# second-state/qwen3_asr_rs

Hardware: NVIDIA H100
Metric: real-time factor (audio-sec/wall-sec) Qwen3-ASR-0.6B 30s clips (higher is better)
Workload: dtype f32 (bf16 weights, fp32-exact activations)

## Files before the change

### qwen3_asr_rs_b200/csrc/attention_f32.cu

```cuda
#include "internal.h"

namespace asrb {

namespace af32 {

static constexpr int QT = 32, KT = 64, THREADS = 128, PS = KT + 4;

template <int HD, bool OFF>
__global__ void __launch_bounds__(THREADS, 2) attn_f32_kernel(AttnParams p) {
    constexpr int NG = HD / 64;
    extern __shared__ __align__(16) float sm[];
    float* Qt = sm;
    float* Kt = Qt + HD * QT;
    float* Vs = Kt + HD * KT;
    float* Ps = Vs + KT * HD;
    const int seg = blockIdx.z, h = blockIdx.y;
    const int q0 = p.seg_q0[seg], len = p.seg_len[seg];
    const int pos0 = OFF ? p.seg_pos0[seg] : 0;
    const int nqt = (len + QT - 1) / QT;
    const int gkv = h / p.group;
    const int tid = threadIdx.x, tx = tid & 15, ty = tid >> 4;
    const float* kbase; const float* vbase;
    if (p.keys_in_rows) {
        kbase = p.k + (size_t)q0 * p.ldk + (size_t)gkv * p.head_stride;
        vbase = p.v + (size_t)q0 * p.ldk + (size_t)gkv * p.head_stride;
    } else {
        kbase = p.k + (size_t)seg * p.seg_stride + (size_t)gkv * p.head_stride;
        vbase = p.v + (size_t)seg * p.seg_stride + (size_t)gkv * p.head_stride;
    }
    const int npass = p.causal ? 2 : 1;
    for (int pass = 0; pass < npass; ++pass) {
// ... 139 lines not shown
    }
}

template <int HD> static size_t smem_bytes() { return (size_t)(HD * QT + HD * KT + KT * HD + QT * PS) * sizeof(float); }

}

bool launch_attention_f32(const AttnParams& p, int hd, cudaStream_t st) {
    using namespace af32;
    if (p.nseg <= 0 || p.max_len <= 0) return true;
    if ((p.ldq % 4) || (p.ldk % 4) || (p.head_stride % 4) || (p.seg_stride % 4)) return false;
    const int nqt_max = (p.max_len + QT - 1) / QT;
    dim3 grid(p.causal ? (nqt_max + 1) / 2 : nqt_max, p.nheads, p.nseg);
    auto run = [&](auto kern, size_t smem) {
        ASRB_CUDA_CHECK(cudaFuncSetAttribute(kern, cudaFuncAttributeMaxDynamicSharedMemorySize, (int)smem));
        kern<<<grid, THREADS, smem, st>>>(p);
    };
    const bool off = p.seg_pos0 != nullptr;
    if (off && !p.causal) return false;
    if (hd == 64) run(off ? attn_f32_kernel<64, true> : attn_f32_kernel<64, false>, smem_bytes<64>());
    else if (hd == 128) run(off ? attn_f32_kernel<128, true> : attn_f32_kernel<128, false>, smem_bytes<128>());
    else return false;
    ASRB_CUDA_CHECK(cudaGetLastError());
    return true;
}

}
```

### qwen3_asr_rs_b200/csrc/common.cuh

```cuda
#pragma once
#include <cuda_runtime.h>
#include <cuda_bf16.h>
#include <stdint.h>
#include <stdexcept>
#include <string>

namespace asrb {

struct Error : public std::runtime_error {
    int code;
    Error(int c, const std::string& m) : std::runtime_error(m), code(c) {}
};

#define ASRB_CUDA_CHECK(expr)                                                              \
    do {                                                                                   \
        cudaError_t _e = (expr);                                                           \
        if (_e != cudaSuccess)                                                             \
            throw ::asrb::Error(2, std::string(#expr) + " failed: " + cudaGetErrorString(_e) + \
                                       " (" __FILE__ ":" + std::to_string(__LINE__) + ")"); \
    } while (0)

#define ASRB_REQUIRE(cond, code, msg)                                          \
    do {                                                                       \
        if (!(cond)) throw ::asrb::Error((code), std::string(msg));            \
// ... 50 lines not shown
    if (lane == 0) scratch[w] = v;
    __syncthreads();
    float r = (lane < nw) ? scratch[lane] : 0.f;
    r = warp_sum(r);
    return r;
}
__device__ __forceinline__ float block_max(float v, float* scratch) {
    int lane = threadIdx.x & 31, w = threadIdx.x >> 5, nw = (blockDim.x + 31) >> 5;
    v = warp_max(v);
    __syncthreads();
    if (lane == 0) scratch[w] = v;
    __syncthreads();
    float r = (lane < nw) ? scratch[lane] : -INFINITY;
    r = warp_max(r);
    return r;
}

__device__ __forceinline__ float lse_rescale(float s, float m, float M) { return m == M ? s : s * expf(m - M); }
__device__ __forceinline__ void lse_fold(float v, int row, float& best_v, int& best_i, float& best_s) {
    if (v > best_v) { best_s = lse_rescale(best_s, best_v, v) + 1.f; best_v = v; best_i = row; }
    else best_s += expf(v - best_v);
}
__device__ __forceinline__ float lse_merge(float m, float s, float om, float os) {
    const float M = fmaxf(m, om);
    return lse_rescale(s, m, M) + lse_rescale(os, om, M);
}

constexpr int TK_MAX = 8;
struct TopK { float v[TK_MAX]; int i[TK_MAX]; };
__device__ __forceinline__ bool tk_before(float a, int ai, float b, int bi) { return a > b || (a == b && ai < bi); }
// ... 146 lines not shown
```

### qwen3_asr_rs_b200/csrc/elementwise.cu

```cuda
#include "internal.h"

namespace asrb {

__global__ void conv1_gelu_kernel(const float* __restrict__ mel, const int* __restrict__ chunk_clip,
                                  const int* __restrict__ chunk_f0, const int64_t* __restrict__ foff,
                                  const int64_t* __restrict__ frames, int n_mels, int W, int OH, int OW,
                                  const float* __restrict__ w, const float* __restrict__ bias, int dsh,
                                  int cpad, bf16* __restrict__ out, size_t plane_stride) {
    extern __shared__ float rows[];
    const int chunk = blockIdx.y, oh = blockIdx.x;
    const int clip = chunk_clip[chunk], f0 = chunk_f0[chunk];
    const int F = (int)frames[clip];
    const float* mp = mel + (size_t)n_mels * foff[clip];
    for (int idx = threadIdx.x; idx < 3 * (W + 2); idx += blockDim.x) {
        int kh = idx / (W + 2), wi = idx - kh * (W + 2);
        int h = 2 * oh + kh - 1, wcol = wi - 1;
        float v = 0.f;
        if (h >= 0 && h < n_mels && wcol >= 0 && wcol < W && f0 + wcol < F) v = mp[(size_t)h * F + f0 + wcol];
        rows[idx] = v;
    }
    __syncthreads();
    const int c = threadIdx.x;
    if (c >= dsh) return;
    float wk[9];
// ... 20 lines not shown
    int W = d.conv_w[0], OH = d.conv_h[1], OW = d.conv_w[1];
    dim3 grid(OH, n_chunks);
    int threads = ((d.c.downsample_hidden_size + 31) / 32) * 32;
    size_t smem = 3 * (W + 2) * sizeof(float);
    conv1_gelu_kernel<<<grid, threads, smem, st>>>(mel, d_chunk_clip, d_chunk_f0, d_foff, d_frames,
                                                   d.c.num_mel_bins, W, OH, OW, m.conv1_w, m.conv1_b,
                                                   d.c.downsample_hidden_size, d.cpad, out_s3, plane_stride);
    ASRB_CUDA_CHECK(cudaGetLastError());
}

__global__ void layernorm_s3_kernel(const float* __restrict__ x, const float* __restrict__ w,
                                    const float* __restrict__ b, int dim, float eps, bf16* __restrict__ out,
                                    size_t plane_stride) {
    __shared__ float red[32];
    const size_t row = blockIdx.x;
    const float* xr = x + row * dim;
    float s = 0.f;
    for (int i = threadIdx.x; i < dim; i += blockDim.x) s += xr[i];
    const float mean = block_sum(s, red) / dim;
    float v = 0.f;
    for (int i = threadIdx.x; i < dim; i += blockDim.x) { float dlt = xr[i] - mean; v = fmaf(dlt, dlt, v); }
    const float var = block_sum(v, red) / dim;
    const float rstd = 1.0f / sqrtf(var + eps);
    for (int i = threadIdx.x; i < dim; i += blockDim.x)
        store_split3(out, plane_stride, row * dim + i, (xr[i] - mean) * rstd * w[i] + b[i]);
}
__global__ void rmsnorm_s3_kernel(const float* __restrict__ x, const float* __restrict__ w, int dim, float eps,
                                  bf16* __restrict__ out, size_t plane_stride) {
    __shared__ float red[32];
    const size_t row = blockIdx.x;
    const float* xr = x + row * dim;
    float s = 0.f;
    for (int i = threadIdx.x; i < dim; i += blockDim.x) s = fmaf(xr[i], xr[i], s);
    const float var = block_sum(s, red) / dim;
    const float r = 1.0f / sqrtf(var + eps);
    for (int i = threadIdx.x; i < dim; i += blockDim.x)
        store_split3(out, plane_stride, row * dim + i, (xr[i] * r) * w[i]);
}
void launch_layernorm_s3(const float* x, const float* w, const float* b, int rows, int dim, float eps,
                         bf16* out_s3, size_t plane_stride, cudaStream_t st) {
    if (rows <= 0) return;
    layernorm_s3_kernel<<<rows, 128, 0, st>>>(x, w, b, dim, eps, out_s3, plane_stride);
    ASRB_CUDA_CHECK(cudaGetLastError());
}
void launch_rmsnorm_s3(const float* x, const float* w, int rows, int dim, float eps, bf16* out_s3,
                       size_t plane_stride, cudaStream_t st) {
    if (rows <= 0) return;
    rmsnorm_s3_kernel<<<rows, 128, 0, st>>>(x, w, dim, eps, out_s3, plane_stride);
    ASRB_CUDA_CHECK(cudaGetLastError());
}

__global__ void embed_inject_kernel(const bf16* __restrict__ embed, int hidden, const int* __restrict__ ids,
                                    const int* __restrict__ audio_row, const float* __restrict__ audio,
                                    float* __restrict__ out) {
    const size_t row = blockIdx.x;
    const int ar = audio_row[row];
    float* o = out + row * hidden;
    if (ar >= 0) {
        const float* a = audio + (size_t)ar * hidden;
        for (int i = threadIdx.x; i < hidden; i += blockDim.x) o[i] = a[i];
    } else {
        const bf16* e = embed + (size_t)ids[row] * hidden;
        for (int i = threadIdx.x; i < hidden; i += blockDim.x) o[i] = __bfloat162float(e[i]);
    }
}
void launch_embed_inject(const bf16* embed, int hidden, const int* d_ids, const int* d_audio_row,
                         const float* audio, int rows, float* out, cudaStream_t st) {
    if (rows <= 0) return;
    embed_inject_kernel<<<rows, 256, 0, st>>>(embed, hidden, d_ids, d_audio_row, audio, out);
    ASRB_CUDA_CHECK(cudaGetLastError());
}

template <bool FAN>
__global__ void qk_norm_rope_kernel(const float* __restrict__ qkv, const int* __restrict__ row_seq,
                                    const int* __restrict__ row_pos, const float* __restrict__ qnorm,
                                    const float* __restrict__ knorm, float eps,
                                    const float* __restrict__ rope_cos, const float* __restrict__ rope_sin,
                                    int nq, int nkv, int hd, float* __restrict__ q_out,
                                    float* __restrict__ kcache, float* __restrict__ vcache,
                                    size_t cache_seq_stride, int max_ctx, FanOut fan) {
    extern __shared__ float sh[];
    float* ys = sh;
    float* red = sh + hd;
    const size_t row = blockIdx.x;
    const int head = blockIdx.y, d = threadIdx.x;
    const int qkv_dim = (nq + 2 * nkv) * hd;
    const float x = qkv[row * qkv_dim + (size_t)head * hd + d];
    const int seq = row_seq[row], pos = row_pos[row];
    const int nfan = FAN && pos < fan.P[seq] ? fan.n[seq] : 0;
    const int* fslots = FAN ? fan.slots + fan.off[seq] : nullptr;
    if (head >= nq + nkv) {
        const size_t o = ((size_t)(head - nq - nkv) * max_ctx + pos) * hd + d;
        vcache[seq * cache_seq_stride + o] = x;
        for (int j = 0; j < nfan; ++j) vcache[(size_t)fslots[j] * cache_seq_stride + o] = x;
        return;
    }
    const float* nw = head < nq ? qnorm : knorm;
    const float var = block_sum(x * x, red) / hd;
    const float y = (x * (1.0f / sqrtf(var + eps))) * nw[d];
    ys[d] = y;
    __syncthreads();
// ... 3 lines not shown
    const float o = y * c + rot * s;
    if (head < nq) q_out[row * ((size_t)nq * hd) + (size_t)head * hd + d] = o;
    else {
        const size_t ko = ((size_t)(head - nq) * max_ctx + pos) * hd + d;
        kcache[seq * cache_seq_stride + ko] = o;
        for (int j = 0; j < nfan; ++j) kcache[(size_t)fslots[j] * cache_seq_stride + ko] = o;
    }
}
void launch_qk_norm_rope(const float* qkv, int rows, const int* d_row_seq, const int* d_row_pos,
                         const float* qnorm, const float* knorm, float eps, const float* rope_cos,
                         const float* rope_sin, int nq, int nkv, int hd, float* q_out, float* kcache,
                         float* vcache, size_t cache_seq_stride, int max_ctx, cudaStream_t st, const FanOut* fan) {
    if (rows <= 0) return;
    dim3 grid(rows, nq + 2 * nkv);
    const size_t smem = (hd + 32) * sizeof(float);
    if (fan) qk_norm_rope_kernel<true><<<grid, hd, smem, st>>>(qkv, d_row_seq, d_row_pos, qnorm, knorm, eps, rope_cos, rope_sin,
                                                               nq, nkv, hd, q_out, kcache, vcache, cache_seq_stride, max_ctx, *fan);
    else qk_norm_rope_kernel<false><<<grid, hd, smem, st>>>(qkv, d_row_seq, d_row_pos, qnorm, knorm, eps, rope_cos, rope_sin,
                                                            nq, nkv, hd, q_out, kcache, vcache, cache_seq_stride, max_ctx, FanOut{});
    ASRB_CUDA_CHECK(cudaGetLastError());
}

}
```

### qwen3_asr_rs_b200/csrc/gemm_simt.cu

```cuda
#include "internal.h"
#include "epilogue.cuh"

namespace asrb {

static constexpr int BM = 64, BN = 64, BK = 16, CHUNK_K = 256;

__global__ void __launch_bounds__(256) gemm_simt_kernel(GemmA A, const bf16* __restrict__ W, int N, GemmEpi E) {
    __shared__ float As[BK][BM + 4];
    __shared__ float Ws[BK][BN + 4];
    const int m0 = blockIdx.y * BM, n0 = blockIdx.x * BN;
    const int tid = threadIdx.x;
    const int tx = tid & 15, ty = tid >> 4;
    float acc[4][4], sum[4][4];
#pragma unroll
    for (int i = 0; i < 4; ++i)
#pragma unroll
        for (int j = 0; j < 4; ++j) acc[i][j] = sum[i][j] = 0.f;
    for (int k0 = 0; k0 < A.K; k0 += BK) {
#pragma unroll
        for (int i = 0; i < 4; ++i) {
            int idx = tid + i * 256;
            int r = idx >> 4, kk = idx & 15;
            int m = m0 + r, k = k0 + kk;
            As[kk][r] = (m < A.M && k < A.K) ? load_a(A, m, k) : 0.f;
// ... 30 lines not shown
            int n = n0 + tx * 4 + j;
            if (n >= N) continue;
            epi_store2(E, N, m, n, sum[i][j], sum[i][j + 1], n + 1 < N);
        }
    }
}

void launch_gemm_simt(const GemmA& A, const bf16* W, int N, const GemmEpi& E, cudaStream_t st) {
    dim3 grid((N + BN - 1) / BN, (A.M + BM - 1) / BM);
    if (A.M <= 0 || N <= 0) return;
    gemm_simt_kernel<<<grid, 256, 0, st>>>(A, W, N, E);
    ASRB_CUDA_CHECK(cudaGetLastError());
}

std::atomic<int64_t> g_gemm_simt_fallbacks{0}, g_gemm_tc_launches{0};

void launch_gemm(const GemmA& A, const bf16* W, int N, const GemmEpi& E, int impl, cudaStream_t st) {
    if (impl == GEMM_TC) {
        if (launch_gemm_tc(A, W, N, E, st)) { g_gemm_tc_launches += 1; return; }
        g_gemm_simt_fallbacks += 1;
    }
    launch_gemm_simt(A, W, N, E, st);
}

}
```

### qwen3_asr_rs_b200/csrc/gemm_tc.cu

```cuda
#include <cuda.h>
#include <algorithm>
#include <cstring>
#include <map>
#include <tuple>
#include "internal.h"
#include "epilogue.cuh"
#include "wgmma.cuh"

namespace asrb {
namespace tc {

static constexpr int BM = 128, BN = 128, BK = 64, STAGES = 3;
static constexpr int TILE_A_BYTES = BM * BK * 2;
static constexpr int TILE_B_BYTES = BN * BK * 2;
static constexpr int STAGE_BYTES = 3 * TILE_A_BYTES + TILE_B_BYTES;
static constexpr int NTHREADS = 384;
static constexpr int CONS_WARPS = 8;
static constexpr int SLAB_LD = 40;
static constexpr int CH = 4;

struct ConvGeom { int OH, OW, box_h, tiles_per_chunk, kblk_per_tap, a_box_bytes; };

template <int A_MODE, int EPI_MODE>
__global__ void __launch_bounds__(NTHREADS, 1)
// ... 2 lines not shown
    extern __shared__ __align__(1024) uint8_t smem_raw[];
    uint8_t* smem = reinterpret_cast<uint8_t*>((reinterpret_cast<uintptr_t>(smem_raw) + 1023) & ~(uintptr_t)1023);
    uint64_t* full = reinterpret_cast<uint64_t*>(smem + STAGES * STAGE_BYTES);
    uint64_t* empty = full + STAGES;
    float* epi_slab = reinterpret_cast<float*>(smem + STAGES * STAGE_BYTES + 256);
    const int warp = threadIdx.x >> 5, lane = threadIdx.x & 31;
    const int num_kb = K / BK / splits;
    const int n_items = tiles_m * tiles_n * splits;

    if (threadIdx.x == 0) {
        for (int i = 0; i < STAGES; ++i) { mbar_init(&full[i], 1); mbar_init(&empty[i], CONS_WARPS); }
        asm volatile("fence.mbarrier_init.release.cluster;" ::: "memory");
        asm volatile("prefetch.tensormap [%0];" ::"l"(&mapA) : "memory");
        asm volatile("prefetch.tensormap [%0];" ::"l"(&mapB) : "memory");
    }
    __syncthreads();

    auto item_coords = [&](int item, int& n0, int& m0, int& chunk, int& oh0, int& z) {
        const int nt = item % tiles_n; int rest = item / tiles_n;
        const int mt = rest % tiles_m; z = rest / tiles_m;
        n0 = nt * BN; m0 = mt * BM; chunk = 0; oh0 = 0;
        if (A_MODE == 1) { chunk = mt / cg.tiles_per_chunk; oh0 = (mt % cg.tiles_per_chunk) * cg.box_h; }
    };

    if (warp == 0 && lane == 0) {
        const uint32_t a_bytes = (A_MODE == 0) ? (uint32_t)TILE_A_BYTES : (uint32_t)cg.a_box_bytes;
        const uint32_t stage_tx = (uint32_t)nplanes * a_bytes + (uint32_t)TILE_B_BYTES;
        uint32_t kg = 0;
        for (int item = blockIdx.x; item < n_items; item += gridDim.x) {
            int n0, m0, chunk, oh0, z;
// ... 51 lines not shown
                    }
                    mr[i] = (m >= 0 && ncol) ? m : -1;
                    if (mr[i] >= 0) in[i] = epi_fetch4<EPI_MODE>(E, N, (int)mr[i], n);
                }
#pragma unroll
                for (int i = 0; i < 4; ++i)
                    if (mr[i] >= 0) epi_store4<EPI_MODE>(E, N, (int)mr[i], n, v[i], bias4, in[i]);
                __syncwarp();
            }
        }
    }
}

template <int MODE>
__global__ void __launch_bounds__(256) splitk_reduce_kernel(const float* __restrict__ ws, int S, int M, int N, GemmEpi E) {
    const int n8 = N / 8;
    const int idx = blockIdx.x * blockDim.x + threadIdx.x;
    if (idx >= M * n8) return;
    const int m = idx / n8, n = (idx - m * n8) * 8;
    float v[8];
#pragma unroll
    for (int i = 0; i < 8; ++i) v[i] = 0.f;
    for (int sp = 0; sp < S; ++sp) {
        const float* src = ws + ((size_t)sp * M + m) * N + n;
        const float4 a = *reinterpret_cast<const float4*>(src), b = *reinterpret_cast<const float4*>(src + 4);
        v[0] += a.x; v[1] += a.y; v[2] += a.z; v[3] += a.w; v[4] += b.x; v[5] += b.y; v[6] += b.z; v[7] += b.w;
    }
    epi_store8<MODE>(E, N, m, n, v);
}

typedef CUresult (*EncodeTiledFn)(CUtensorMap*, CUtensorMapDataType, cuuint32_t, void*, const cuuint64_t*, const cuuint64_t*,
                                  const cuuint32_t*, const cuuint32_t*, CUtensorMapInterleave, CUtensorMapSwizzle,
                                  CUtensorMapL2promotion, CUtensorMapFloatOOBfill);
static EncodeTiledFn get_encode() {
    static EncodeTiledFn fn = nullptr;
    if (!fn) {
        void* p = nullptr;
        cudaDriverEntryPointQueryResult qr;
        ASRB_CUDA_CHECK(cudaGetDriverEntryPoint("cuTensorMapEncodeTiled", &p, cudaEnableDefault, &qr));
        ASRB_REQUIRE(p != nullptr && qr == cudaDriverEntryPointSuccess, ASRB_ERR_CUDA, "cuTensorMapEncodeTiled unavailable");
        fn = (EncodeTiledFn)p;
    }
    return fn;
// ... 91 lines not shown
    cuuint64_t bs[1] = {(cuuint64_t)A.K * 2};
    cuuint32_t bb[2] = {(cuuint32_t)BK, (cuuint32_t)BN};
    const CUtensorMap mapB = cached_map(W, 2, bd, bs, bb);
    ConvGeom cg{};
    const size_t smem = smem_bytes();
    const int tiles_m = pl.tiles_m, tiles_n = pl.tiles_n;
    if (A.mode == A_PLAIN) {
        cuuint64_t ad[3] = {(cuuint64_t)A.K, (cuuint64_t)A.M, (cuuint64_t)3};
        cuuint64_t as[2] = {(cuuint64_t)A.lda * 2, (cuuint64_t)A.plane_stride * 2};
        cuuint32_t ab[3] = {(cuuint32_t)BK, (cuuint32_t)BM, 1};
        const CUtensorMap mapA = cached_map(A.a, 3, ad, as, ab);
        if (pl.splits > 1) {
            GemmEpi P;
            P.out_f32 = E.splitk_ws; P.ldo = N;
            ASRB_CUDA_CHECK(cudaFuncSetAttribute(gemm_tc_kernel<0, EPI_PLAIN>, cudaFuncAttributeMaxDynamicSharedMemorySize, (int)smem));
            gemm_tc_kernel<0, EPI_PLAIN><<<pl.grid, NTHREADS, smem, st>>>(mapA, mapB, A.M, N, A.K, A.nplanes, tiles_m, tiles_n, pl.splits, cg, P);
            const int work = A.M * (N / 8);
            if (E.mode == EPI_PLAIN) splitk_reduce_kernel<EPI_PLAIN><<<(work + 255) / 256, 256, 0, st>>>(E.splitk_ws, pl.splits, A.M, N, E);
            else splitk_reduce_kernel<EPI_CONVOUT><<<(work + 255) / 256, 256, 0, st>>>(E.splitk_ws, pl.splits, A.M, N, E);
            ASRB_CUDA_CHECK(cudaGetLastError());
            if (E.extra_launches) *E.extra_launches += 1;
            return true;
        }
#define ASRB_TC_LAUNCH(AM, EM)                                                                                         \
    {                                                                                                                  \
        ASRB_CUDA_CHECK(cudaFuncSetAttribute(gemm_tc_kernel<AM, EM>, cudaFuncAttributeMaxDynamicSharedMemorySize, (int)smem)); \
        gemm_tc_kernel<AM, EM><<<pl.grid, NTHREADS, smem, st>>>(mapA, mapB, A.M, N, A.K, A.nplanes, tiles_m, tiles_n, 1, cg, E); \
    }
        if (E.mode == EPI_PLAIN) ASRB_TC_LAUNCH(0, EPI_PLAIN)
        else if (E.mode == EPI_SWIGLU) ASRB_TC_LAUNCH(0, EPI_SWIGLU)
        else ASRB_TC_LAUNCH(0, EPI_CONVOUT)
    } else {
        const int chunks = A.M / (A.OH * A.OW);
        cg.OH = A.OH; cg.OW = A.OW; cg.box_h = pl.box_h;
        cg.tiles_per_chunk = (A.OH + cg.box_h - 1) / cg.box_h; cg.kblk_per_tap = A.cpad / BK;
        cg.a_box_bytes = A.OW * cg.box_h * BK * 2;
        cuuint64_t ad[5] = {(cuuint64_t)A.cpad, (cuuint64_t)A.Wh, (cuuint64_t)A.Hh, (cuuint64_t)chunks * 4, 3};
        cuuint64_t as[4] = {(cuuint64_t)A.cpad * 2, (cuuint64_t)A.Wh * A.cpad * 2, (cuuint64_t)A.Hh * A.Wh * A.cpad * 2,
                            (cuuint64_t)A.plane_stride * 2};
        cuuint32_t ab[5] = {(cuuint32_t)BK, (cuuint32_t)A.OW, (cuuint32_t)cg.box_h, 1, 1};
        const CUtensorMap mapA = cached_map(A.a, 5, ad, as, ab);
        if (E.mode == EPI_CONV_PARITY) ASRB_TC_LAUNCH(1, EPI_CONV_PARITY)
        else ASRB_TC_LAUNCH(1, EPI_CONV_FEAT)
#undef ASRB_TC_LAUNCH
    }
    ASRB_CUDA_CHECK(cudaGetLastError());
    return true;
}

}
```

### qwen3_asr_rs_b200/csrc/internal.h

```cpp
#pragma once
#include <atomic>
#include <map>
#include <string>
#include <vector>
#include "../../include/asr_b200.h"
#include "common.cuh"

namespace asrb {

struct Dims {
    asrb_dims c;
    int enc_hd;
    int chunk_frames;
    int chunks_per_window;
    int conv_h[4];
    int conv_w[4];
    int tok_per_chunk;
    int cpad;
    int feat;
    int q_dim, kv_dim, qkv_dim;
    void derive();
};
void validate_dims(const asrb_dims& d);
inline int conv_out_len(int l) { return (l - 1) / 2 + 1; }
// ... 51 lines not shown
    int rope_max_pos = 0;

    ~Model();
};

enum { A_PLAIN = 0, A_CONV = 1 };
struct GemmA {
    int mode = A_PLAIN;
    const bf16* a = nullptr;
    size_t plane_stride = 0;
    int nplanes = 3;
    int M = 0, K = 0, lda = 0;
    int OH = 0, OW = 0, Hh = 0, Wh = 0, cpad = 0;
};
enum { EPI_PLAIN = 0, EPI_SWIGLU = 1, EPI_CONV_PARITY = 2, EPI_CONV_FEAT = 3, EPI_CONVOUT = 4 };
struct GemmEpi {
    int mode = EPI_PLAIN;
    const float* bias = nullptr;
    int act = 0;
    const float* residual = nullptr;
    int ldr = 0;
    float* out_f32 = nullptr;
    int ldo = 0;
    bf16* out_s3 = nullptr;
    size_t s3_plane_stride = 0;
    int lds = 0;
    int OH = 0, OW = 0, Hh2 = 0, Wh2 = 0, cpad = 0;
    const int* row_map = nullptr;
    const float* pos = nullptr;
    int pos_period = 1;
    float* splitk_ws = nullptr;
    int64_t* extra_launches = nullptr;
};
static constexpr size_t SPLITK_WS_FLOATS = (size_t)4 * 64 * 128 * 128;
enum { GEMM_SIMT = 0, GEMM_TC = 1 };
extern std::atomic<int64_t> g_gemm_simt_fallbacks, g_gemm_tc_launches;
void launch_gemm(const GemmA& A, const bf16* W, int N, const GemmEpi& E, int impl, cudaStream_t st);
bool launch_gemm_tc(const GemmA& A, const bf16* W, int N, const GemmEpi& E, cudaStream_t st);
struct GemmPlan { bool tc = false; int splits = 1, tiles_m = 0, tiles_n = 0, grid = 0, box_h = 0; };
GemmPlan plan_gemm_tc(const GemmA& A, int N, const GemmEpi& E, int sms);
void launch_gemm_simt(const GemmA& A, const bf16* W, int N, const GemmEpi& E, cudaStream_t st);

void launch_mel(const Model& m, const float* samples, const int64_t* d_soff, const int64_t* d_n,
                const int64_t* d_npad, const int64_t* d_foff, int batch, int max_frames,
                float* mel_out, int* d_maxkey, cudaStream_t st);
void launch_mel_stream(const Model& m, const float* samples, const int64_t* d_soff, const int64_t* d_n, const int64_t* d_npad,
                       const int64_t* d_foff, const int* d_ffirst, int n_streams, int max_new_frames, int ldo, float* raw,
                       const int4* d_fold, int win_frames, float* stats, int stats_ld, cudaStream_t st);
void launch_mel_stream_stage(const Model& m, const float* raw, const int4* d_plan, const int64_t* d_foff, int n_utt, int ldo,
                             float* mel_out, cudaStream_t st);
void launch_segment(const float* d_long, const int64_t* d_plan, int n_files, int64_t total_blocks, int64_t max_seg,
                    int64_t search, double* d_blk, int64_t* d_cuts, int64_t* d_ncuts, int sm_count, cudaStream_t st);
void launch_conv1(const Model& m, const float* mel, const int* d_chunk_clip, const int* d_chunk_f0,
                  const int64_t* d_foff, const int64_t* d_frames, int n_chunks,
                  bf16* out_s3, size_t plane_stride, cudaStream_t st);
void launch_layernorm_s3(const float* x, const float* w, const float* b, int rows, int dim, float eps,
                         bf16* out_s3, size_t plane_stride, cudaStream_t st);
void launch_rmsnorm_s3(const float* x, const float* w, int rows, int dim, float eps,
                       bf16* out_s3, size_t plane_stride, cudaStream_t st);
void launch_embed_inject(const bf16* embed, int hidden, const int* d_ids, const int* d_audio_row,
                         const float* audio, int rows, float* out, cudaStream_t st);
struct FanOut {
    const int* n;
    const int* off;
    const int* P;
    const int* slots;
};
void launch_qk_norm_rope(const float* qkv, int rows, const int* d_row_seq, const int* d_row_pos,
                         const float* qnorm, const float* knorm, float eps,
                         const float* rope_cos, const float* rope_sin,
                         int nq, int nkv, int hd, float* q_out, float* kcache, float* vcache,
                         size_t cache_seq_stride, int max_ctx, cudaStream_t st, const FanOut* fan = nullptr);
struct AttnParams {
    const float* q; int ldq;
// ... 109 lines not shown
```

### qwen3_asr_rs_b200/csrc/probe.cu

```cuda
#include <algorithm>
#include <functional>
#include <vector>
#include "internal.h"
#include "probe.h"

namespace asrb {
int run_guarded(const std::function<void()>& f);
bool launch_attention_f32(const AttnParams& p, int hd, cudaStream_t st);

namespace {

struct Scope {
    cudaStream_t st = nullptr;
    std::vector<void*> bufs;
    Scope() { ASRB_CUDA_CHECK(cudaStreamCreateWithFlags(&st, cudaStreamNonBlocking)); }
    ~Scope() {
        if (st) cudaStreamSynchronize(st);
        for (void* p : bufs) cudaFree(p);
        if (st) cudaStreamDestroy(st);
    }
    template <typename T> T* alloc(size_t n, int fill_byte = 0) {
        void* p = nullptr;
        ASRB_CUDA_CHECK(cudaMalloc(&p, std::max<size_t>(n, 1) * sizeof(T)));
        bufs.push_back(p);
// ... 36 lines not shown
}

GemmA plan_operand(int M, int K, int a_mode, int OH, int OW, int cpad, size_t plane_stride) {
    GemmA A; A.mode = a_mode; A.M = M; A.K = K; A.lda = K; A.nplanes = 3; A.plane_stride = plane_stride;
    A.OH = OH; A.OW = OW; A.Hh = OH; A.Wh = OW; A.cpad = cpad;
    return A;
}
size_t round8(size_t n) { return (n + 7) / 8 * 8; }

}
}

using namespace asrb;

extern "C" {

int asrbt_split3(const float* x, int64_t n, uint16_t* planes_out) {
    return run_guarded([&] {
        ASRB_REQUIRE(x && planes_out && n >= 0, ASRB_ERR_INVALID, "asrbt_split3: bad arguments");
        Scope s;
        float* d_x = s.upload(x, (size_t)n);
        bf16* d_p = s.alloc<bf16>(3 * (size_t)n);
        split3_planes(s, d_x, (size_t)n, d_p, (size_t)n);
        s.download(planes_out, reinterpret_cast<const uint16_t*>(d_p), 3 * (size_t)n);
        s.sync();
    });
}

int asrbt_norm_s3(int kind, const float* x, const float* w, const float* b, int rows, int dim, float eps, uint16_t* planes_out) {
    return run_guarded([&] {
// ... 125 lines not shown
```

### qwen3_asr_rs_b200/csrc/probe.h

```cpp
#ifndef ASR_B200_PROBE_H
#define ASR_B200_PROBE_H
#include <stdint.h>
#include "../../include/asr_b200.h"

#ifdef __cplusplus
extern "C" {
#endif

#define ASRBT_PLAN_LEN 8

typedef struct {
    int impl;
    int a_mode;
    int epi;
    int M, N, K, nplanes;
    const float* x;
    int OH, OW, Hh, Wh, cpad;
    const uint16_t* w;
    const float* bias;
    int gelu;
    const float* residual;
    const int* row_map;
    const float* pos;
    int pos_period;
    int use_splitk;
    float* out_f32; int64_t out_f32_rows; int ldo;
    uint16_t* out_planes; int64_t out_plane_elems; int lds;
    int Hh2, Wh2, cpad2;
} asrbt_gemm_args;

typedef struct {
    int hd, nseg, nheads, group, causal, keys_in_rows, max_len;
    const int* seg_q0; const int* seg_len; const int* seg_pos0;
    const float* buf; int64_t buf_elems;
    int64_t q_off, k_off, v_off;
    int ldq, ldk; int64_t seg_stride, head_stride;
    uint16_t* out_planes; int64_t out_rows; int ldo;
} asrbt_attn_args;

ASRB_API int asrbt_split3(const float* x, int64_t n, uint16_t* planes_out);
ASRB_API int asrbt_norm_s3(int kind, const float* x, const float* w, const float* b, int rows, int dim, float eps,
                           uint16_t* planes_out);
ASRB_API int asrbt_gemm_plan(int M, int N, int K, int a_mode, int epi, int sms, int use_splitk, int OH, int OW, int cpad,
                             int* plan_out);
ASRB_API int asrbt_gemm(const asrbt_gemm_args* a, int* plan_out);
ASRB_API int asrbt_attention(const asrbt_attn_args* a);

#ifdef __cplusplus
}
#endif
#endif
```

### qwen3_asr_rs_b200/csrc/session.cu

```cuda
#include <algorithm>
#include <cerrno>
#include <cmath>
#include <cstdlib>
#include <cstring>
#include <limits>
#include "internal.h"

namespace asrb {

void model_set_tensor(Model* m, const char* name, int dtype, const int64_t* shape, int ndim, const void* host);
void model_finalize(Model* m);
struct IngestState;
IngestState* ingest_state_new();
void ingest_state_free(IngestState* st);
void ingest_pcm(IngestState* st, cudaStream_t stream, const void* const* pcm, const int64_t* n_frames, const int32_t* channels,
                const int32_t* rate, const int32_t* format, int batch, float* d_samples, int64_t max_samples_per_utt,
                int64_t* n_out, int64_t* soff_out);

static const int kPromptHead[9] = {151644, 8948, 198, 151645, 198, 151644, 872, 198, 151669};
static const int kPromptTail[6] = {151670, 151645, 198, 151644, 77091, 198};
static const int kAudioPad = 151676;

struct Session {
    Model* m = nullptr;
// ... 445 lines not shown
        A.OH = d.conv_h[3]; A.OW = d.conv_w[3]; A.Hh = d.conv_h[3]; A.Wh = d.conv_w[3]; A.cpad = d.cpad;
        A.M = totC * A.OH * A.OW; A.K = 9 * d.cpad; A.lda = A.K;
        GemmEpi E; E.mode = EPI_CONV_FEAT; E.bias = m.conv3_b; E.out_s3 = s->feat; E.s3_plane_stride = s->feat_ps;
        E.OH = A.OH; E.OW = A.OW; E.lds = d.feat;
        launch_gemm(A, m.conv3_w, c.downsample_hidden_size, E, s->gemm_impl, st);
    }
    {
        GemmA A = plainA(s->feat, s->feat_ps, totC * tpc, d.feat, np);
        GemmEpi E; E.mode = EPI_CONVOUT; E.bias = m.conv_out_b; E.out_f32 = s->x_enc; E.ldo = c.d_model;
        E.splitk_ws = s->splitk_ws; E.extra_launches = &s->launches;
        E.row_map = s->d_rowmap; E.pos = m.pos_emb; E.pos_period = tpc;
        launch_gemm(A, m.conv_out_w, c.d_model, E, s->gemm_impl, st);
    }
    s->launches += 4;
    const int dm = c.d_model;
    for (int l = 0; l < c.encoder_layers; ++l) {
        const EncLayerW& w = m.enc[l];
        launch_layernorm_s3(s->x_enc, w.ln1_w, w.ln1_b, totT, dm, 1e-5f, s->enc_h, s->ench_ps, st);
        { GemmA A = plainA(s->enc_h, s->ench_ps, totT, dm, np);
          GemmEpi E; E.bias = w.bqkv; E.out_f32 = s->enc_qkv; E.ldo = 3 * dm;
          launch_gemm(A, w.wqkv, 3 * dm, E, s->gemm_impl, st); }
        { AttnParams p{}; p.q = s->enc_qkv; p.ldq = 3 * dm; p.k = s->enc_qkv + dm; p.v = s->enc_qkv + 2 * dm;
          p.head_stride = d.enc_hd; p.ldk = 3 * dm; p.seg_stride = 0; p.keys_in_rows = 1;
          p.seg_q0 = s->d_win_q0; p.seg_len = s->d_win_len; p.nseg = nwin; p.nheads = c.encoder_attention_heads; p.group = 1;
          p.causal = 0; p.max_len = maxwin; p.out_s3 = s->enc_attn; p.plane_stride = s->ench_ps; p.ldo = dm;
          launch_attention(p, d.enc_hd, st); }
        { GemmA A = plainA(s->enc_attn, s->ench_ps, totT, dm, np);
          GemmEpi E; E.bias = w.bo; E.residual = s->x_enc; E.ldr = dm; E.out_f32 = s->x_enc; E.ldo = dm; E.splitk_ws = s->splitk_ws; E.extra_launches = &s->launches;
          launch_gemm(A, w.wo, dm, E, s->gemm_impl, st); }
        launch_layernorm_s3(s->x_enc, w.ln2_w, w.ln2_b, totT, dm, 1e-5f, s->enc_h, s->ench_ps, st);
        { GemmA A = plainA(s->enc_h, s->ench_ps, totT, dm, np);
          GemmEpi E; E.bias = w.b1; E.act = 1; E.out_s3 = s->enc_ff; E.s3_plane_stride = s->encff_ps; E.lds = c.encoder_ffn_dim;
          launch_gemm(A, w.fc1, c.encoder_ffn_dim, E, s->gemm_impl, st); }
        { GemmA A = plainA(s->enc_ff, s->encff_ps, totT, c.encoder_ffn_dim, np);
          GemmEpi E; E.bias = w.b2; E.residual = s->x_enc; E.ldr = dm; E.out_f32 = s->x_enc; E.ldo = dm; E.splitk_ws = s->splitk_ws; E.extra_launches = &s->launches;
          launch_gemm(A, w.fc2, dm, E, s->gemm_impl, st); }
        s->launches += 7;
    }
    launch_layernorm_s3(s->x_enc, m.lnpost_w, m.lnpost_b, totT, dm, 1e-5f, s->enc_h, s->ench_ps, st);
    { GemmA A = plainA(s->enc_h, s->ench_ps, totT, dm, np);
      GemmEpi E; E.bias = m.proj1_b; E.act = 1; E.out_s3 = s->enc_attn; E.s3_plane_stride = s->ench_ps; E.lds = dm;
      launch_gemm(A, m.proj1, dm, E, s->gemm_impl, st); }
    { GemmA A = plainA(s->enc_attn, s->ench_ps, totT, dm, np);
      GemmEpi E; E.bias = m.proj2_b; E.out_f32 = s->audio; E.ldo = c.output_dim; E.splitk_ws = s->splitk_ws; E.extra_launches = &s->launches;
      launch_gemm(A, m.proj2, c.output_dim, E, s->gemm_impl, st); }
    s->launches += 3;
    if (n_tokens_out) for (int b = 0; b < B; ++b) n_tokens_out[b] = s->T[b];
    s->stage = 2;
}

void session_encode_read(Session* s, int b, float* out) {
    ASRB_REQUIRE(s->stage >= 2 && !s->stream_run && b >= 0 && b < s->B, ASRB_ERR_STATE, "encode_read: nothing encoded for this index");
    ASRB_CUDA_CHECK(cudaStreamSynchronize(s->st));
    const int od = s->m->d.c.output_dim;
    ASRB_CUDA_CHECK(cudaMemcpy(out, s->audio + (size_t)s->toff[b] * od, (size_t)s->T[b] * od * sizeof(float), cudaMemcpyDeviceToHost));
}

static void check_sampling_options(const Session* s, int batch) {
    ASRB_REQUIRE(!(s->temperature > 0.0 && s->top_k > 0), ASRB_ERR_INVALID, "temperature > 0 cannot be combined with top_logprobs");
    if (s->beam_k > 1) {
        ASRB_REQUIRE(s->temperature == 0.0, ASRB_ERR_INVALID, "beam_size > 1 cannot be combined with temperature > 0");
// ... 85 lines not shown
    const int nl = s->S[b] - (15 + (int)cb.size() + s->T[b]);
    build_prompt(cb, s->T[b], s->toff[b], nl > 0 ? lang_ids[b] : nullptr, nl, {}, pid, parow);
}
static int plan_prompt_rows(const std::vector<int>& pid, const std::vector<int>& parow, int from, int r0, int q, int* ids,
                            int* arow, int* rseq, int* rpos) {
    int r = r0;
    for (int i = from; i < (int)pid.size(); ++i, ++r) { ids[r] = pid[i]; arow[r] = parow[i]; rseq[r] = q; rpos[r] = i; }
    return r;
}

static void prefill_layers(Session* s, int totS, int nseq, int maxrows, const FanOut* fan, const int* d_qpos0,
                           const float* audio) {
    Model& m = *s->m; const Dims& d = m.d; const asrb_dims& c = d.c;
    cudaStream_t st = s->st; const int np = s->nplanes;
    launch_embed_inject(m.embed, c.hidden_size, s->d_ids, s->d_audio_row, audio, totS, s->hid, st);
    s->launches += 1;
    const int H = c.hidden_size; const float eps = (float)c.rms_norm_eps;
    for (int l = 0; l < c.num_hidden_layers; ++l) {
        const DecLayerW& w = m.dec[l];
        float* kc = s->kcache + (size_t)l * s->cache_layer_stride;
        float* vc = s->vcache + (size_t)l * s->cache_layer_stride;
        launch_rmsnorm_s3(s->hid, w.ln_in, totS, H, eps, s->dh, s->dh_ps, st);
        { GemmA A = plainA(s->dh, s->dh_ps, totS, H, np);
          GemmEpi E; E.out_f32 = s->dqkv; E.ldo = d.qkv_dim;
          launch_gemm(A, w.wqkv, d.qkv_dim, E, s->gemm_impl, st); }
        launch_qk_norm_rope(s->dqkv, totS, s->d_row_seq, s->d_row_pos, w.qnorm, w.knorm, eps, m.rope_cos, m.rope_sin,
                            c.num_attention_heads, c.num_key_value_heads, c.head_dim, s->qrot, kc, vc, s->cache_seq_stride,
                            s->max_ctx, st, fan);
        { AttnParams p{}; p.q = s->qrot; p.ldq = d.q_dim; p.k = kc; p.v = vc; p.seg_stride = s->cache_seq_stride;
          p.head_stride = (size_t)s->max_ctx * c.head_dim; p.ldk = c.head_dim; p.keys_in_rows = 0;
          p.seg_q0 = s->d_seq_q0; p.seg_len = s->d_seq_len; p.nseg = nseq; p.nheads = c.num_attention_heads;
          p.group = c.num_attention_heads / c.num_key_value_heads; p.causal = 1; p.max_len = maxrows; p.seg_pos0 = d_qpos0;
          p.out_s3 = s->dattn; p.plane_stride = s->dattn_ps; p.ldo = d.q_dim;
          launch_attention(p, c.head_dim, st); }
        { GemmA A = plainA(s->dattn, s->dattn_ps, totS, d.q_dim, np);
          GemmEpi E; E.residual = s->hid; E.ldr = H; E.out_f32 = s->hid; E.ldo = H; E.splitk_ws = s->splitk_ws; E.extra_launches = &s->launches;
          launch_gemm(A, w.wo, H, E, s->gemm_impl, st); }
        launch_rmsnorm_s3(s->hid, w.ln_post, totS, H, eps, s->dh, s->dh_ps, st);
        { GemmA A = plainA(s->dh, s->dh_ps, totS, H, np);
          GemmEpi E; E.mode = EPI_SWIGLU; E.out_s3 = s->dact; E.s3_plane_stride = s->dact_ps; E.lds = c.intermediate_size;
          launch_gemm(A, w.wgu, 2 * c.intermediate_size, E, s->gemm_impl, st); }
        { GemmA A = plainA(s->dact, s->dact_ps, totS, c.intermediate_size, np);
          GemmEpi E; E.residual = s->hid; E.ldr = H; E.out_f32 = s->hid; E.ldo = H; E.splitk_ws = s->splitk_ws; E.extra_launches = &s->launches;
          launch_gemm(A, w.wdown, H, E, s->gemm_impl, st); }
        s->launches += 8;
    }
}

static void begin_run(Session* s, int B, const int* d_done0);
static void first_token(Session* s, int B, bool write_logits, const int* pos0);

void session_prefill(Session* s, const int64_t* const* lang_ids, const int32_t* n_lang_ids, int64_t* seq_lens_out,
                     float* last_logits) {
    ASRB_REQUIRE(s->stage >= 2 && !s->stream_run, ASRB_ERR_STATE, "prefill called before encode");
    check_sampling_options(s, s->B);
    s->streams_open = false;
    check_context(s, s->B);
    Model& m = *s->m; const asrb_dims& c = m.d.c;
    const int B = s->B; cudaStream_t st = s->st;
    for (int b = 0; b < B; ++b) {
// ... 1010 lines not shown
```

Baseline: 332.9.

## Fuse split-K reduce with following norm and enable programmatic dependent launch

```diff
diff --git a/qwen3_asr_rs_b200/csrc/attention_f32.cu b/qwen3_asr_rs_b200/csrc/attention_f32.cu
--- a/qwen3_asr_rs_b200/csrc/attention_f32.cu
+++ b/qwen3_asr_rs_b200/csrc/attention_f32.cu
@@ -15,6 +15,7 @@
     float* Vs = Kt + HD * KT;
     float* Ps = Vs + KT * HD;
     const int seg = blockIdx.z, h = blockIdx.y;
+    pdl_enter();
     const int q0 = p.seg_q0[seg], len = p.seg_len[seg];
     const int pos0 = OFF ? p.seg_pos0[seg] : 0;
     const int nqt = (len + QT - 1) / QT;
@@ -184,7 +185,7 @@
     dim3 grid(p.causal ? (nqt_max + 1) / 2 : nqt_max, p.nheads, p.nseg);
     auto run = [&](auto kern, size_t smem) {
         ASRB_CUDA_CHECK(cudaFuncSetAttribute(kern, cudaFuncAttributeMaxDynamicSharedMemorySize, (int)smem));
-        kern<<<grid, THREADS, smem, st>>>(p);
+        launch_pdl(kern, grid, dim3(THREADS), smem, st, p);
     };
     const bool off = p.seg_pos0 != nullptr;
     if (off && !p.causal) return false;
diff --git a/qwen3_asr_rs_b200/csrc/common.cuh b/qwen3_asr_rs_b200/csrc/common.cuh
--- a/qwen3_asr_rs_b200/csrc/common.cuh
+++ b/qwen3_asr_rs_b200/csrc/common.cuh
@@ -88,6 +88,31 @@
     float r = (lane < nw) ? scratch[lane] : -INFINITY;
     r = warp_max(r);
     return r;
+}
+
+__device__ __forceinline__ void pdl_enter() { asm volatile("griddepcontrol.wait;" ::: "memory"); }
+
+__device__ __forceinline__ void layernorm_row_s3(const float* xr, const float* __restrict__ w, const float* __restrict__ b,
+                                                 int dim, float eps, bf16* __restrict__ out, size_t plane_stride, size_t row,
+                                                 float* red) {
+    float s = 0.f;
+    for (int i = threadIdx.x; i < dim; i += blockDim.x) s += xr[i];
+    const float mean = block_sum(s, red) / dim;
+    float v = 0.f;
+    for (int i = threadIdx.x; i < dim; i += blockDim.x) { float dlt = xr[i] - mean; v = fmaf(dlt, dlt, v); }
+    const float var = block_sum(v, red) / dim;
+    const float rstd = 1.0f / sqrtf(var + eps);
+    for (int i = threadIdx.x; i < dim; i += blockDim.x)
+        store_split3(out, plane_stride, row * dim + i, (xr[i] - mean) * rstd * w[i] + b[i]);
+}
+__device__ __forceinline__ void rmsnorm_row_s3(const float* xr, const float* __restrict__ w, int dim, float eps,
+                                               bf16* __restrict__ out, size_t plane_stride, size_t row, float* red) {
+    float s = 0.f;
+    for (int i = threadIdx.x; i < dim; i += blockDim.x) s = fmaf(xr[i], xr[i], s);
+    const float var = block_sum(s, red) / dim;
+    const float r = 1.0f / sqrtf(var + eps);
+    for (int i = threadIdx.x; i < dim; i += blockDim.x)
+        store_split3(out, plane_stride, row * dim + i, (xr[i] * r) * w[i]);
 }
 
 __device__ __forceinline__ float lse_rescale(float s, float m, float M) { return m == M ? s : s * expf(m - M); }
diff --git a/qwen3_asr_rs_b200/csrc/elementwise.cu b/qwen3_asr_rs_b200/csrc/elementwise.cu
--- a/qwen3_asr_rs_b200/csrc/elementwise.cu
+++ b/qwen3_asr_rs_b200/csrc/elementwise.cu
@@ -58,46 +58,41 @@
                                     size_t plane_stride) {
     __shared__ float red[32];
     const size_t row = blockIdx.x;
-    const float* xr = x + row * dim;
-    float s = 0.f;
-    for (int i = threadIdx.x; i < dim; i += blockDim.x) s += xr[i];
-    const float mean = block_sum(s, red) / dim;
-    float v = 0.f;
-    for (int i = threadIdx.x; i < dim; i += blockDim.x) { float dlt = xr[i] - mean; v = fmaf(dlt, dlt, v); }
-    const float var = block_sum(v, red) / dim;
-    const float rstd = 1.0f / sqrtf(var + eps);
-    for (int i = threadIdx.x; i < dim; i += blockDim.x)
-        store_split3(out, plane_stride, row * dim + i, (xr[i] - mean) * rstd * w[i] + b[i]);
+    pdl_enter();
+    layernorm_row_s3(x + row * dim, w, b, dim, eps, out, plane_stride, row, red);
 }
 __global__ void rmsnorm_s3_kernel(const float* __restrict__ x, const float* __restrict__ w, int dim, float eps,
                                   bf16* __restrict__ out, size_t plane_stride) {
     __shared__ float red[32];
     const size_t row = blockIdx.x;
-    const float* xr = x + row * dim;
-    float s = 0.f;
-    for (int i = threadIdx.x; i < dim; i += blockDim.x) s = fmaf(xr[i], xr[i], s);
-    const float var = block_sum(s, red) / dim;
-    const float r = 1.0f / sqrtf(var + eps);
-    for (int i = threadIdx.x; i < dim; i += blockDim.x)
-        store_split3(out, plane_stride, row * dim + i, (xr[i] * r) * w[i]);
+    pdl_enter();
+    rmsnorm_row_s3(x + row * dim, w, dim, eps, out, plane_stride, row, red);
 }
 void launch_layernorm_s3(const float* x, const float* w, const float* b, int rows, int dim, float eps,
                          bf16* out_s3, size_t plane_stride, cudaStream_t st) {
     if (rows <= 0) return;
-    layernorm_s3_kernel<<<rows, 128, 0, st>>>(x, w, b, dim, eps, out_s3, plane_stride);
+    launch_pdl(layernorm_s3_kernel, dim3(rows), dim3(128), 0, st, x, w, b, dim, eps, out_s3, plane_stride);
     ASRB_CUDA_CHECK(cudaGetLastError());
 }
 void launch_rmsnorm_s3(const float* x, const float* w, int rows, int dim, float eps, bf16* out_s3,
                        size_t plane_stride, cudaStream_t st) {
     if (rows <= 0) return;
-    rmsnorm_s3_kernel<<<rows, 128, 0, st>>>(x, w, dim, eps, out_s3, plane_stride);
+    launch_pdl(rmsnorm_s3_kernel, dim3(rows), dim3(128), 0, st, x, w, dim, eps, out_s3, plane_stride);
     ASRB_CUDA_CHECK(cudaGetLastError());
+}
+void launch_norm_s3(const GemmEpi& E, int rows, int dim, cudaStream_t st) {
+    const NormS3& n = E.norm;
+    if (n.kind == NORM_NONE) return;
+    if (n.kind == NORM_LAYER) launch_layernorm_s3(E.out_f32, n.w, n.b, rows, dim, n.eps, n.out, n.plane_stride, st);
+    else launch_rmsnorm_s3(E.out_f32, n.w, rows, dim, n.eps, n.out, n.plane_stride, st);
+    if (E.extra_launches) *E.extra_launches += 1;
 }
 
 __global__ void embed_inject_kernel(const bf16* __restrict__ embed, int hidden, const int* __restrict__ ids,
                                     const int* __restrict__ audio_row, const float* __restrict__ audio,
                                     float* __restrict__ out) {
     const size_t row = blockIdx.x;
+    pdl_enter();
     const int ar = audio_row[row];
     float* o = out + row * hidden;
     if (ar >= 0) {
@@ -111,7 +106,7 @@
 void launch_embed_inject(const bf16* embed, int hidden, const int* d_ids, const int* d_audio_row,
                          const float* audio, int rows, float* out, cudaStream_t st) {
     if (rows <= 0) return;
-    embed_inject_kernel<<<rows, 256, 0, st>>>(embed, hidden, d_ids, d_audio_row, audio, out);
+    launch_pdl(embed_inject_kernel, dim3(rows), dim3(256), 0, st, embed, hidden, d_ids, d_audio_row, audio, out);
     ASRB_CUDA_CHECK(cudaGetLastError());
 }
 
@@ -129,6 +124,7 @@
     const size_t row = blockIdx.x;
     const int head = blockIdx.y, d = threadIdx.x;
     const int qkv_dim = (nq + 2 * nkv) * hd;
+    pdl_enter();
     const float x = qkv[row * qkv_dim + (size_t)head * hd + d];
     const int seq = row_seq[row], pos = row_pos[row];
     const int nfan = FAN && pos < fan.P[seq] ? fan.n[seq] : 0;
@@ -162,10 +158,9 @@
     if (rows <= 0) return;
     dim3 grid(rows, nq + 2 * nkv);
     const size_t smem = (hd + 32) * sizeof(float);
-    if (fan) qk_norm_rope_kernel<true><<<grid, hd, smem, st>>>(qkv, d_row_seq, d_row_pos, qnorm, knorm, eps, rope_cos, rope_sin,
-                                                               nq, nkv, hd, q_out, kcache, vcache, cache_seq_stride, max_ctx, *fan);
-    else qk_norm_rope_kernel<false><<<grid, hd, smem, st>>>(qkv, d_row_seq, d_row_pos, qnorm, knorm, eps, rope_cos, rope_sin,
-                                                            nq, nkv, hd, q_out, kcache, vcache, cache_seq_stride, max_ctx, FanOut{});
+    launch_pdl(fan ? qk_norm_rope_kernel<true> : qk_norm_rope_kernel<false>, grid, dim3(hd), smem, st, qkv, d_row_seq, d_row_pos,
+               qnorm, knorm, eps, rope_cos, rope_sin, nq, nkv, hd, q_out, kcache, vcache, cache_seq_stride, max_ctx,
+               fan ? *fan : FanOut{});
     ASRB_CUDA_CHECK(cudaGetLastError());
 }
 
diff --git a/qwen3_asr_rs_b200/csrc/gemm_simt.cu b/qwen3_asr_rs_b200/csrc/gemm_simt.cu
--- a/qwen3_asr_rs_b200/csrc/gemm_simt.cu
+++ b/qwen3_asr_rs_b200/csrc/gemm_simt.cu
@@ -68,6 +68,7 @@
 }
 
 std::atomic<int64_t> g_gemm_simt_fallbacks{0}, g_gemm_tc_launches{0};
+std::atomic<int> g_fuse_splitk_norm{1}, g_pdl{1};
 
 void launch_gemm(const GemmA& A, const bf16* W, int N, const GemmEpi& E, int impl, cudaStream_t st) {
     if (impl == GEMM_TC) {
@@ -75,6 +76,7 @@
         g_gemm_simt_fallbacks += 1;
     }
     launch_gemm_simt(A, W, N, E, st);
+    launch_norm_s3(E, A.M, N, st);
 }
 
 }
diff --git a/qwen3_asr_rs_b200/csrc/gemm_tc.cu b/qwen3_asr_rs_b200/csrc/gemm_tc.cu
--- a/qwen3_asr_rs_b200/csrc/gemm_tc.cu
+++ b/qwen3_asr_rs_b200/csrc/gemm_tc.cu
@@ -40,6 +40,7 @@
         asm volatile("prefetch.tensormap [%0];" ::"l"(&mapA) : "memory");
         asm volatile("prefetch.tensormap [%0];" ::"l"(&mapB) : "memory");
     }
+    pdl_enter();
     __syncthreads();
 
     auto item_coords = [&](int item, int& n0, int& m0, int& chunk, int& oh0, int& z) {
@@ -121,6 +122,7 @@
 
 template <int MODE>
 __global__ void __launch_bounds__(256) splitk_reduce_kernel(const float* __restrict__ ws, int S, int M, int N, GemmEpi E) {
+    pdl_enter();
     const int n8 = N / 8;
     const int idx = blockIdx.x * blockDim.x + threadIdx.x;
     if (idx >= M * n8) return;
@@ -134,6 +136,23 @@
         v[0] += a.x; v[1] += a.y; v[2] += a.z; v[3] += a.w; v[4] += b.x; v[5] += b.y; v[6] += b.z; v[7] += b.w;
     }
     epi_store8<MODE>(E, N, m, n, v);
+}
+
+template <int NORM>
+__global__ void __launch_bounds__(128) splitk_reduce_norm_kernel(const float* __restrict__ ws, int S, int M, int N, GemmEpi E) {
+    __shared__ float red[32];
+    const int m = blockIdx.x;
+    pdl_enter();
+    float* xr = E.out_f32 + (size_t)m * E.ldo;
+    for (int n = threadIdx.x; n < N; n += blockDim.x) {
+        float v = 0.f;
+        for (int sp = 0; sp < S; ++sp) v += ws[((size_t)sp * M + m) * N + n];
+        if (E.bias) v += E.bias[n];
+        if (E.residual) v += E.residual[(size_t)m * E.ldr + n];
+        xr[n] = v;
+    }
+    if (NORM == NORM_LAYER) layernorm_row_s3(xr, E.norm.w, E.norm.b, N, E.norm.eps, E.norm.out, E.norm.plane_stride, m, red);
+    else rmsnorm_row_s3(xr, E.norm.w, N, E.norm.eps, E.norm.out, E.norm.plane_stride, m, red);
 }
 
 typedef CUresult (*EncodeTiledFn)(CUtensorMap*, CUtensorMapDataType, cuuint32_t, void*, const cuuint64_t*, const cuuint64_t*,
@@ -255,18 +274,26 @@
             GemmEpi P;
             P.out_f32 = E.splitk_ws; P.ldo = N;
             ASRB_CUDA_CHECK(cudaFuncSetAttribute(gemm_tc_kernel<0, EPI_PLAIN>, cudaFuncAttributeMaxDynamicSharedMemorySize, (int)smem));
-            gemm_tc_kernel<0, EPI_PLAIN><<<pl.grid, NTHREADS, smem, st>>>(mapA, mapB, A.M, N, A.K, A.nplanes, tiles_m, tiles_n, pl.splits, cg, P);
+            launch_pdl(gemm_tc_kernel<0, EPI_PLAIN>, dim3(pl.grid), dim3(NTHREADS), smem, st, mapA, mapB, A.M, N, A.K, A.nplanes, tiles_m, tiles_n, pl.splits, cg, P);
             const int work = A.M * (N / 8);
-            if (E.mode == EPI_PLAIN) splitk_reduce_kernel<EPI_PLAIN><<<(work + 255) / 256, 256, 0, st>>>(E.splitk_ws, pl.splits, A.M, N, E);
-            else splitk_reduce_kernel<EPI_CONVOUT><<<(work + 255) / 256, 256, 0, st>>>(E.splitk_ws, pl.splits, A.M, N, E);
+            const bool fuse = E.norm.kind != NORM_NONE && g_fuse_splitk_norm.load() && E.mode == EPI_PLAIN && E.act == 0 &&
+                              E.out_f32 && E.ldo == N && !E.out_s3;
+            if (fuse)
+                launch_pdl(E.norm.kind == NORM_LAYER ? splitk_reduce_norm_kernel<NORM_LAYER> : splitk_reduce_norm_kernel<NORM_RMS>,
+                           dim3(A.M), dim3(128), 0, st, E.splitk_ws, pl.splits, A.M, N, E);
+            else
+                launch_pdl(E.mode == EPI_PLAIN ? splitk_reduce_kernel<EPI_PLAIN> : splitk_reduce_kernel<EPI_CONVOUT>,
+                           dim3((work + 255) / 256), dim3(256), 0, st, E.splitk_ws, pl.splits, A.M, N, E);
             ASRB_CUDA_CHECK(cudaGetLastError());
             if (E.extra_launches) *E.extra_launches += 1;
+            if (!fuse) launch_norm_s3(E, A.M, N, st);
             return true;
         }
 #define ASRB_TC_LAUNCH(AM, EM)                                                                                         \
     {                                                                                                                  \
         ASRB_CUDA_CHECK(cudaFuncSetAttribute(gemm_tc_kernel<AM, EM>, cudaFuncAttributeMaxDynamicSharedMemorySize, (int)smem)); \
-        gemm_tc_kernel<AM, EM><<<pl.grid, NTHREADS, smem, st>>>(mapA, mapB, A.M, N, A.K, A.nplanes, tiles_m, tiles_n, 1, cg, E); \
+        launch_pdl(gemm_tc_kernel<AM, EM>, dim3(pl.grid), dim3(NTHREADS), smem, st, mapA, mapB, A.M, N, A.K, A.nplanes,   \
+                   tiles_m, tiles_n, 1, cg, E);                                                                         \
     }
         if (E.mode == EPI_PLAIN) ASRB_TC_LAUNCH(0, EPI_PLAIN)
         else if (E.mode == EPI_SWIGLU) ASRB_TC_LAUNCH(0, EPI_SWIGLU)
@@ -286,6 +313,7 @@
 #undef ASRB_TC_LAUNCH
     }
     ASRB_CUDA_CHECK(cudaGetLastError());
+    launch_norm_s3(E, A.M, N, st);
     return true;
 }
 
diff --git a/qwen3_asr_rs_b200/csrc/internal.h b/qwen3_asr_rs_b200/csrc/internal.h
--- a/qwen3_asr_rs_b200/csrc/internal.h
+++ b/qwen3_asr_rs_b200/csrc/internal.h
@@ -1,5 +1,6 @@
 #pragma once
 #include <atomic>
+#include <utility>
 #include <map>
 #include <string>
 #include <vector>
@@ -89,6 +90,15 @@
     int OH = 0, OW = 0, Hh = 0, Wh = 0, cpad = 0;
 };
 enum { EPI_PLAIN = 0, EPI_SWIGLU = 1, EPI_CONV_PARITY = 2, EPI_CONV_FEAT = 3, EPI_CONVOUT = 4 };
+enum { NORM_NONE = 0, NORM_LAYER = 1, NORM_RMS = 2 };
+struct NormS3 {
+    int kind = NORM_NONE;
+    const float* w = nullptr;
+    const float* b = nullptr;
+    float eps = 0.f;
+    bf16* out = nullptr;
+    size_t plane_stride = 0;
+};
 struct GemmEpi {
     int mode = EPI_PLAIN;
     const float* bias = nullptr;
@@ -106,6 +116,7 @@
     int pos_period = 1;
     float* splitk_ws = nullptr;
     int64_t* extra_launches = nullptr;
+    NormS3 norm;
 };
 static constexpr size_t SPLITK_WS_FLOATS = (size_t)4 * 64 * 128 * 128;
 enum { GEMM_SIMT = 0, GEMM_TC = 1 };
@@ -133,6 +144,19 @@
                          bf16* out_s3, size_t plane_stride, cudaStream_t st);
 void launch_rmsnorm_s3(const float* x, const float* w, int rows, int dim, float eps,
                        bf16* out_s3, size_t plane_stride, cudaStream_t st);
+void launch_norm_s3(const GemmEpi& E, int rows, int dim, cudaStream_t st);
+extern std::atomic<int> g_pdl;
+template <typename... KArgs, typename... Args>
+void launch_pdl(void (*kern)(KArgs...), dim3 grid, dim3 block, size_t smem, cudaStream_t st, Args&&... args) {
+    cudaLaunchConfig_t cfg = {};
+    cfg.gridDim = grid; cfg.blockDim = block; cfg.dynamicSmemBytes = smem; cfg.stream = st;
+    cudaLaunchAttribute at[1];
+    at[0].id = cudaLaunchAttributeProgrammaticStreamSerialization;
+    at[0].val.programmaticStreamSerializationAllowed = 1;
+    cfg.attrs = at; cfg.numAttrs = g_pdl.load() ? 1 : 0;
+    ASRB_CUDA_CHECK(cudaLaunchKernelEx(&cfg, kern, std::forward<Args>(args)...));
+}
+extern std::atomic<int> g_fuse_splitk_norm;
 void launch_embed_inject(const bf16* embed, int hidden, const int* d_ids, const int* d_audio_row,
                          const float* audio, int rows, float* out, cudaStream_t st);
 struct FanOut {
diff --git a/qwen3_asr_rs_b200/csrc/probe.cu b/qwen3_asr_rs_b200/csrc/probe.cu
--- a/qwen3_asr_rs_b200/csrc/probe.cu
+++ b/qwen3_asr_rs_b200/csrc/probe.cu
@@ -74,6 +74,14 @@
 using namespace asrb;
 
 extern "C" {
+
+int asrbt_set_fused_norm(int on) {
+    return run_guarded([&] { g_fuse_splitk_norm.store(on ? 1 : 0); });
+}
+
+int asrbt_set_pdl(int on) {
+    return run_guarded([&] { g_pdl.store(on ? 1 : 0); });
+}
 
 int asrbt_split3(const float* x, int64_t n, uint16_t* planes_out) {
     return run_guarded([&] {
diff --git a/qwen3_asr_rs_b200/csrc/probe.h b/qwen3_asr_rs_b200/csrc/probe.h
--- a/qwen3_asr_rs_b200/csrc/probe.h
+++ b/qwen3_asr_rs_b200/csrc/probe.h
@@ -38,6 +38,8 @@
     uint16_t* out_planes; int64_t out_rows; int ldo;
 } asrbt_attn_args;
 
+ASRB_API int asrbt_set_fused_norm(int on);
+ASRB_API int asrbt_set_pdl(int on);
 ASRB_API int asrbt_split3(const float* x, int64_t n, uint16_t* planes_out);
 ASRB_API int asrbt_norm_s3(int kind, const float* x, const float* w, const float* b, int rows, int dim, float eps,
                            uint16_t* planes_out);
diff --git a/qwen3_asr_rs_b200/csrc/session.cu b/qwen3_asr_rs_b200/csrc/session.cu
--- a/qwen3_asr_rs_b200/csrc/session.cu
+++ b/qwen3_asr_rs_b200/csrc/session.cu
@@ -483,9 +483,14 @@
     }
     s->launches += 4;
     const int dm = c.d_model;
+    auto enc_norm = [&](const float* w, const float* b) {
+        NormS3 n; n.kind = NORM_LAYER; n.w = w; n.b = b; n.eps = 1e-5f; n.out = s->enc_h; n.plane_stride = s->ench_ps;
+        return n;
+    };
+    launch_layernorm_s3(s->x_enc, m.enc[0].ln1_w, m.enc[0].ln1_b, totT, dm, 1e-5f, s->enc_h, s->ench_ps, st);
+    s->launches += 1;
     for (int l = 0; l < c.encoder_layers; ++l) {
         const EncLayerW& w = m.enc[l];
-        launch_layernorm_s3(s->x_enc, w.ln1_w, w.ln1_b, totT, dm, 1e-5f, s->enc_h, s->ench_ps, st);
         { GemmA A = plainA(s->enc_h, s->ench_ps, totT, dm, np);
           GemmEpi E; E.bias = w.bqkv; E.out_f32 = s->enc_qkv; E.ldo = 3 * dm;
           launch_gemm(A, w.wqkv, 3 * dm, E, s->gemm_impl, st); }
@@ -496,24 +501,24 @@
           launch_attention(p, d.enc_hd, st); }
         { GemmA A = plainA(s->enc_attn, s->ench_ps, totT, dm, np);
           GemmEpi E; E.bias = w.bo; E.residual = s->x_enc; E.ldr = dm; E.out_f32 = s->x_enc; E.ldo = dm; E.splitk_ws = s->splitk_ws; E.extra_launches = &s->launches;
+          E.norm = enc_norm(w.ln2_w, w.ln2_b);
           launch_gemm(A, w.wo, dm, E, s->gemm_impl, st); }
-        launch_layernorm_s3(s->x_enc, w.ln2_w, w.ln2_b, totT, dm, 1e-5f, s->enc_h, s->ench_ps, st);
         { GemmA A = plainA(s->enc_h, s->ench_ps, totT, dm, np);
           GemmEpi E; E.bias = w.b1; E.act = 1; E.out_s3 = s->enc_ff; E.s3_plane_stride = s->encff_ps; E.lds = c.encoder_ffn_dim;
           launch_gemm(A, w.fc1, c.encoder_ffn_dim, E, s->gemm_impl, st); }
         { GemmA A = plainA(s->enc_ff, s->encff_ps, totT, c.encoder_ffn_dim, np);
           GemmEpi E; E.bias = w.b2; E.residual = s->x_enc; E.ldr = dm; E.out_f32 = s->x_enc; E.ldo = dm; E.splitk_ws = s->splitk_ws; E.extra_launches = &s->launches;
+          E.norm = l + 1 < c.encoder_layers ? enc_norm(m.enc[l + 1].ln1_w, m.enc[l + 1].ln1_b) : enc_norm(m.lnpost_w, m.lnpost_b);
           launch_gemm(A, w.fc2, dm, E, s->gemm_impl, st); }
-        s->launches += 7;
-    }
-    launch_layernorm_s3(s->x_enc, m.lnpost_w, m.lnpost_b, totT, dm, 1e-5f, s->enc_h, s->ench_ps, st);
+        s->launches += 5;
+    }
     { GemmA A = plainA(s->enc_h, s->ench_ps, totT, dm, np);
       GemmEpi E; E.bias = m.proj1_b; E.act = 1; E.out_s3 = s->enc_attn; E.s3_plane_stride = s->ench_ps; E.lds = dm;
       launch_gemm(A, m.proj1, dm, E, s->gemm_impl, st); }
     { GemmA A = plainA(s->enc_attn, s->ench_ps, totT, dm, np);
       GemmEpi E; E.bias = m.proj2_b; E.out_f32 = s->audio; E.ldo = c.output_dim; E.splitk_ws = s->splitk_ws; E.extra_launches = &s->launches;
       launch_gemm(A, m.proj2, c.output_dim, E, s->gemm_impl, st); }
-    s->launches += 3;
+    s->launches += 2;
     if (n_tokens_out) for (int b = 0; b < B; ++b) n_tokens_out[b] = s->T[b];
     s->stage = 2;
 }
@@ -629,13 +634,17 @@
     Model& m = *s->m; const Dims& d = m.d; const asrb_dims& c = d.c;
     cudaStream_t st = s->st; const int np = s->nplanes;
     launch_embed_inject(m.embed, c.hidden_size, s->d_ids, s->d_audio_row, audio, totS, s->hid, st);
-    s->launches += 1;
     const int H = c.hidden_size; const float eps = (float)c.rms_norm_eps;
+    auto dec_norm = [&](const float* w) {
+        NormS3 n; n.kind = NORM_RMS; n.w = w; n.eps = eps; n.out = s->dh; n.plane_stride = s->dh_ps;
+        return n;
+    };
+    launch_rmsnorm_s3(s->hid, m.dec[0].ln_in, totS, H, eps, s->dh, s->dh_ps, st);
+    s->launches += 2;
     for (int l = 0; l < c.num_hidden_layers; ++l) {
         const DecLayerW& w = m.dec[l];
         float* kc = s->kcache + (size_t)l * s->cache_layer_stride;
         float* vc = s->vcache + (size_t)l * s->cache_layer_stride;
-        launch_rmsnorm_s3(s->hid, w.ln_in, totS, H, eps, s->dh, s->dh_ps, st);
         { GemmA A = plainA(s->dh, s->dh_ps, totS, H, np);
           GemmEpi E; E.out_f32 = s->dqkv; E.ldo = d.qkv_dim;
           launch_gemm(A, w.wqkv, d.qkv_dim, E, s->gemm_impl, st); }
@@ -650,15 +659,16 @@
           launch_attention(p, c.head_dim, st); }
         { GemmA A = plainA(s->dattn, s->dattn_ps, totS, d.q_dim, np);
           GemmEpi E; E.residual = s->hid; E.ldr = H; E.out_f32 = s->hid; E.ldo = H; E.splitk_ws = s->splitk_ws; E.extra_launches = &s->launches;
+          E.norm = dec_norm(w.ln_post);
           launch_gemm(A, w.wo, H, E, s->gemm_impl, st); }
-        launch_rmsnorm_s3(s->hid, w.ln_post, totS, H, eps, s->dh, s->dh_ps, st);
         { GemmA A = plainA(s->dh, s->dh_ps, totS, H, np);
           GemmEpi E; E.mode = EPI_SWIGLU; E.out_s3 = s->dact; E.s3_plane_stride = s->dact_ps; E.lds = c.intermediate_size;
           launch_gemm(A, w.wgu, 2 * c.intermediate_size, E, s->gemm_impl, st); }
         { GemmA A = plainA(s->dact, s->dact_ps, totS, c.intermediate_size, np);
           GemmEpi E; E.residual = s->hid; E.ldr = H; E.out_f32 = s->hid; E.ldo = H; E.splitk_ws = s->splitk_ws; E.extra_launches = &s->launches;
+          if (l + 1 < c.num_hidden_layers) E.norm = dec_norm(m.dec[l + 1].ln_in);
           launch_gemm(A, w.wdown, H, E, s->gemm_impl, st); }
-        s->launches += 8;
+        s->launches += 6;
     }
 }
 
```

Result: no change. 335.3, median of 6 (+0.7%).
